# HI-ComputerVision/uni-encoder-code

Measured on AMD Instinct MI355X. Metric: img/s fwd+bwd Swin-L 1024x2048 bs=2 per GPU, higher is better.
Workload: dtype bf16; 1 GPU; BASELINE configs[2]: full OneFormer (Swin-L ws12 backbone + MSDeformAttn pixel decoder + 150-query masked-attention decoder), 1024x2048, fwd+bwd, synthetic loss; global_batch=2, parallelism=dp1, mode=eval() (train_mode reported separately with --full)

## Files before the change

include/uenc.h:

```cpp
#ifndef UENC_H
#define UENC_H
#include <stdint.h>

#ifdef __cplusplus
extern "C" {
#endif

#define UENC_F32 0
#define UENC_BF16 1

#ifndef UENC_STREAM_T
#define UENC_STREAM_T void*
#endif
typedef UENC_STREAM_T uenc_stream_t;

#define UENC_EPI_NONE 0
#define UENC_EPI_GELU 1
#define UENC_EPI_RELU 2
#define UENC_EPI_RESIDUAL 3
#define UENC_EPI_MUL_DGELU 4
#define UENC_EPI_MUL_DRELU 5

int uenc_version(void);
const char* uenc_arch(void);

int uenc_cast_f32_bf16(const float* src, void* dst, long n , uenc_stream_t stream);
int uenc_dropout_bf16(const void* in, void* out, long n, unsigned seed, float p, uenc_stream_t stream);
int uenc_cast_transpose_f32_bf16(const float* src , void* dst , int R, int C, uenc_stream_t stream);

int uenc_cast_multi(const void* table, int n, long total_tiles, uenc_stream_t stream);

int uenc_upsample_bilinear(const float* in, float* out, long NC, int Hi, int Wi, int Ho, int Wo, uenc_stream_t stream);

int uenc_attn_mask(const float* logits, uint8_t* mask, long rows, int Hi, int Wi, int Ho, int Wo, uenc_stream_t stream);

int uenc_add_cast_bf16(const float* a, const float* b, void* out, long n, long period, uenc_stream_t stream);
int uenc_msda_prep_fwd(const float* offaw, long ld, const float* ref, int ref_per_image, const int64_t* shapes, float* loc,
                       float* aw, long rows, int Lq, int M, int L, int P, uenc_stream_t stream);
int uenc_msda_prep_bwd(const float* dloc, const float* daw, const float* aw, const int64_t* shapes, void* doffaw, long ld,
                       long rows, int Lq, int M, int L, int P, uenc_stream_t stream);
int uenc_segment_colsum(const void* x16, long ld, int cols, const int64_t* seg_start, int nseg, long rows_per_image, int images,
                        float* out, uenc_stream_t stream);
// ... 287 lines not shown
```

uni-encoder-code_amd/csrc/fpn_nearest.hip:

```cpp
#include "common.h"

struct NrP {
    const void* a; int a_f32;
    const void* prev; int prev_f32;
    void* out; int out_f32;
    const void* dy; int dy_f32;
    float* dprev;
    int B, H, W, Hs, Ws, C;
};

__device__ __forceinline__ float4 nr_ld4(const void* base, int is_f32, long idx) {
    if (is_f32) return *(const float4*)((const float*)base + idx);
    const bf16x4 v = *(const bf16x4*)((const bf16*)base + idx);
    return make_float4((float)v[0], (float)v[1], (float)v[2], (float)v[3]);
}

__device__ __forceinline__ int nearest_src(int dst, float scale, int n_in) { return min((int)floorf((float)dst * scale), n_in - 1); }

__global__ __launch_bounds__(256) void merge_nearest_fwd_kernel(NrP p) {
    const int cqn = p.C >> 2;
    const long total = (long)p.B * p.H * p.W * cqn;
    const float sy = (float)p.Hs / (float)p.H, sx = (float)p.Ws / (float)p.W;
    for (long t = (long)blockIdx.x * 256 + threadIdx.x; t < total; t += (long)gridDim.x * 256) {
        const int cq = (int)(t % cqn);
// ... 20 lines not shown
    if (i == n_in - 1) hi = n_out - 1;
    lo = lo < 0 ? 0 : lo;
    hi = hi > n_out - 1 ? n_out - 1 : hi;
}

__global__ __launch_bounds__(256) void merge_nearest_bwd_kernel(NrP p) {
    const int cqn = p.C >> 2;
    const long total = (long)p.B * p.Hs * p.Ws * cqn;
    const float sy = (float)p.Hs / (float)p.H, sx = (float)p.Ws / (float)p.W;
    for (long t = (long)blockIdx.x * 256 + threadIdx.x; t < total; t += (long)gridDim.x * 256) {
        const int cq = (int)(t % cqn);
        long r = t / cqn;
        const int j = (int)(r % p.Ws); r /= p.Ws;
        const int i = (int)(r % p.Hs);
        const int b = (int)(r / p.Hs);
        int ylo, yhi, xlo, xhi;
        nearest_range(i, p.Hs, p.H, sy, ylo, yhi);
        nearest_range(j, p.Ws, p.W, sx, xlo, xhi);
        float4 acc = make_float4(0.f, 0.f, 0.f, 0.f);
        for (int oy = ylo; oy <= yhi; ++oy) {
            if (nearest_src(oy, sy, p.Hs) != i) continue;
            for (int ox = xlo; ox <= xhi; ++ox) {
                if (nearest_src(ox, sx, p.Ws) != j) continue;
                const float4 d = nr_ld4(p.dy, p.dy_f32, (((long)b * p.H + oy) * p.W + ox) * p.C + cq * 4);
                acc.x += d.x; acc.y += d.y; acc.z += d.z; acc.w += d.w;
            }
        }
        *(float4*)(p.dprev + t * 4) = acc;
    }
}

static bool nr_dtype(int d) { return d == UENC_F32 || d == UENC_BF16; }

extern "C" int uenc_merge_nearest_tokens_fwd(const void* a, int a_dtype, const void* prev, int prev_dtype, void* out, int out_dtype, int B,
                                             int H, int W, int Hs, int Ws, int C, hipStream_t stream) {
    UENC_CHECK_ARG(a && prev && out && B > 0 && H > 0 && W > 0 && Hs > 0 && Ws > 0 && C > 0 && C % 4 == 0);
    UENC_CHECK_ARG(nr_dtype(a_dtype) && nr_dtype(prev_dtype) && nr_dtype(out_dtype));
    UENC_CHECK_ARG(((uintptr_t)a & (a_dtype == UENC_F32 ? 15 : 7)) == 0 && ((uintptr_t)prev & (prev_dtype == UENC_F32 ? 15 : 7)) == 0 &&
                   ((uintptr_t)out & (out_dtype == UENC_F32 ? 15 : 7)) == 0);
    NrP p{a, a_dtype == UENC_F32, prev, prev_dtype == UENC_F32, out, out_dtype == UENC_F32, nullptr, 0, nullptr, B, H, W, Hs, Ws, C};
    const long total = (long)B * H * W * (C / 4);
    long blocks = (total + 255) / 256;
    if (blocks > 16384) blocks = 16384;
    hipLaunchKernelGGL(merge_nearest_fwd_kernel, dim3((unsigned)blocks), dim3(256), 0, stream, p);
    UENC_LAUNCH_RET();
}

extern "C" int uenc_merge_nearest_tokens_bwd(const void* dy, int dy_dtype, float* dprev, int B, int H, int W, int Hs, int Ws, int C,
                                             hipStream_t stream) {
    UENC_CHECK_ARG(dy && dprev && B > 0 && H > 0 && W > 0 && Hs > 0 && Ws > 0 && C > 0 && C % 4 == 0);
    UENC_CHECK_ARG(nr_dtype(dy_dtype) && ((uintptr_t)dy & (dy_dtype == UENC_F32 ? 15 : 7)) == 0 && ((uintptr_t)dprev & 15) == 0);
    NrP p{nullptr, 0, nullptr, 0, nullptr, 0, dy, dy_dtype == UENC_F32, dprev, B, H, W, Hs, Ws, C};
    const long total = (long)B * Hs * Ws * (C / 4);
    long blocks = (total + 255) / 256;
    if (blocks > 16384) blocks = 16384;
    hipLaunchKernelGGL(merge_nearest_bwd_kernel, dim3((unsigned)blocks), dim3(256), 0, stream, p);
    UENC_LAUNCH_RET();
}
```

uni-encoder-code_amd/csrc/gemm.hip:

```cpp
#include "common.h"
#include "prof.h"

#define BM 128
#define BN 128
#define BK 64
#define GEMM_THREADS 256

enum { EPI_NONE = 0, EPI_GELU = 1, EPI_RELU = 2, EPI_RESIDUAL = 3, EPI_MUL_DGELU = 4, EPI_MUL_DRELU = 5 };

struct GemmNT {
    const void* A; int a_f32; long lda;
    const bf16* W; long ldw;
    void* C; long ldc;
    const float* bias;
    const void* aux; long ldaux;
    bf16* aux_out; long ldaux_out;
    int M, N, K;
    int tiles_m, tiles_n;
    int klen;
    int atomic;
    int persist;
    float alpha;
    const float* sample_scale; float inv_rows;
    long part_stride;
    int splits;
    long bsA, bsW, bsC;
    const float* ln_gamma; const float* ln_beta; float* ln_y32; bf16* ln_y16; float2* ln_stats; float ln_eps;
};

__device__ __forceinline__ float nt_alpha(const GemmNT& p, int m) {
    return p.sample_scale == nullptr ? p.alpha : p.alpha * p.sample_scale[(int)(((float)m + 0.5f) * p.inv_rows)];
}

__device__ __forceinline__ int lds_off(int row, int chunk) { return row * 128 + ((chunk ^ ((row >> 1) & 7)) << 4); }

template <bool F32>
__device__ __forceinline__ u32x4 load_row8(const void* base, long ld, int row, int nrows, int k, int kend, int K) {
    const bool ok = (row < nrows) && (k < kend);
    const int rc = min(row, nrows - 1), kc = min(k, K - 8);
    u32x4 v;
    if (F32) {
        const float* p = (const float*)base + (long)rc * ld + kc;
        const float4 a = *(const float4*)p, b = *(const float4*)(p + 4);
        const bf16x8 r = cvt8(a, b);
        v = *(const u32x4*)&r;
    } else {
        v = *(const u32x4*)((const bf16*)base + (long)rc * ld + kc);
    }
    const u32x4 z = {0u, 0u, 0u, 0u};
    return ok ? v : z;
}

template <int EPI, int OUT_F32>
__global__ __launch_bounds__(GEMM_THREADS) void gemm_nt_kernel(GemmNT p) {
    __shared__ __attribute__((aligned(16))) unsigned char smem[2 * (BM + BN) * BK * 2];
    if (blockIdx.z > 0) {
        p.A = (const char*)p.A + (long)blockIdx.z * p.bsA * (p.a_f32 ? 4 : 2);
        p.W += (long)blockIdx.z * p.bsW;
        p.C = (char*)p.C + (long)blockIdx.z * p.bsC * (OUT_F32 ? 4 : 2);
    }
// ... 621 lines not shown
                bf16x8 sv;
                if (full8) sv = *(const bf16x8*)ap;
                else {
                    const bf16x4 q4 = *(const bf16x4*)ap;
#pragma unroll
                    for (int r = 0; r < 4; ++r) { sv[r] = q4[r]; sv[4 + r] = (bf16)0.f; }
                }
#pragma unroll
                for (int r = 0; r < 8; ++r)
                    v[r] = (EPI == EPI_MUL_DGELU) ? v[r] * dgelu_f((float)sv[r]) : (((float)sv[r] > 0.f) ? v[r] : 0.f);
            }
            if (OUT_F32) {
                float* c = (float*)p.C + (long)m * p.ldc + n;
                if (EPI == EPI_NONE && p.atomic) {
#pragma unroll
                    for (int r = 0; r < 8; ++r)
                        if (r < 4 || full8) atomicAdd(c + r, v[r]);
                } else {
                    *(float4*)c = make_float4(v[0], v[1], v[2], v[3]);
                    if (full8) *(float4*)(c + 4) = make_float4(v[4], v[5], v[6], v[7]);
                }
            } else {
                bf16x8 o;
#pragma unroll
                for (int r = 0; r < 8; ++r) o[r] = (bf16)v[r];
                bf16* c = (bf16*)p.C + (long)m * p.ldc + n;
                if (full8) *(bf16x8*)c = o;
                else { bf16x4 q4; q4[0] = o[0]; q4[1] = o[1]; q4[2] = o[2]; q4[3] = o[3]; *(bf16x4*)c = q4; }
            }
        }
    }
}

template <int EPI, int OUT_F32, int BNT = BN2, bool LN = false>
__global__ __launch_bounds__(T2) void gemm_nt256_kernel(GemmNT p) {
    static_assert(BNT == 256 || BNT == 192, "tile width");
    constexpr int NI = BNT / 64;
    constexpr int NB1 = NI - 2;
    constexpr int BNW = BNT / 4;
    extern __shared__ __attribute__((aligned(16))) unsigned char smem[];
    const int t = threadIdx.x, lane = t & 63, wave = t >> 6;
    const int wm = wave >> 2, wn = wave & 3;
    const int ntiles_all = p.tiles_m * p.tiles_n;
    int pos = blockIdx.x;
    bool prefetched = false;
    const bf16* src[4][2];
    for (;;) {
    const int tile = xcd_remap(pos, ntiles_all);
    const int mt = tile / p.tiles_n, nt = tile - mt * p.tiles_n;
    const int m0 = mt * BM2, n0 = nt * BNT;
    const int pos_next = pos + (int)gridDim.x;
    const bool has_next = p.persist && pos_next < ntiles_all;
    const int kt0 = blockIdx.y * (p.klen / BK);
    const int nkt = min(p.K / BK - kt0, p.klen / BK);
    if (OUT_F32 && p.part_stride > 0) p.C = (float*)p.C + (long)blockIdx.y * p.part_stride;

    f32x4 acc[4][8];
#pragma unroll
    for (int i = 0; i < 4; ++i)
#pragma unroll
        for (int j = 0; j < 8; ++j) acc[i][j] = (f32x4){0.f, 0.f, 0.f, 0.f};

    typedef __attribute__((address_space(3))) void lds_void;
    const int fr = lane & 15, fg = lane >> 4;
    {
        auto set_src = [&](int mm0, int nn0) {
#pragma unroll
            for (int q = 0; q < 2; ++q) {
                const int lr = q * 64 + (t >> 3), slot = t & 7;
                const int chunk = slot ^ ((lr >> 1) & 7);
                const int ra = (lr >> 6) * 128 + (lr & 63), rb = (lr >> 5) * BNW + (lr & 31);
                const int rb1 = NB1 == 2 ? rb + 32 : (lr >> 4) * BNW + 32 + (lr & 15);
                src[0][q] = (const bf16*)p.A + (long)min(mm0 + ra, p.M - 1) * p.lda + chunk * 8 + (long)kt0 * BK;
                src[3][q] = (const bf16*)p.A + (long)min(mm0 + ra + 64, p.M - 1) * p.lda + chunk * 8 + (long)kt0 * BK;
                src[1][q] = p.W + (long)min(nn0 + rb, p.N - 1) * p.ldw + chunk * 8 + (long)kt0 * BK;
                src[2][q] = p.W + (long)min(nn0 + rb1, p.N - 1) * p.ldw + chunk * 8 + (long)kt0 * BK;
            }
        };
        if (!prefetched) set_src(m0, n0);
        const int U = 4 * nkt;
        auto issue = [&](int o, int tile) {
            unsigned char* dst = smem + (tile & 1) * 65536 + (o == 0 ? 0 : o == 1 ? 32768 : o == 2 ? 49152 : 16384) + wave * 1024;
#pragma unroll
            for (int q = 0; q < 2; ++q)
                if (q == 0 || o != 2 || NB1 == 2)
                    __builtin_amdgcn_global_load_lds(src[o][q] + (long)tile * BK, (lds_void*)(dst + q * 8192), 16, 0, 0);
        };
        auto inflight = [&](int first) {
            if (NB1 == 2) return 2 * min(max(U - first, 0), 4);
            int n = 0;
#pragma unroll
            for (int k = 0; k < 4; ++k)
                if (first + k < U) n += (((first + k) & 3) == 2) ? 1 : 2;
            return n;
        };
        auto prologue = [&]() {
            if (BNT == 192) { issue(0, 0); issue(1, 0); issue(3, 0); issue(2, 0); }
            else { issue(0, 0); issue(1, 0); issue(2, 0); issue(3, 0); }
            if (U > 4) { issue(0, 1); issue(1, 1); }
        };
        if (!prefetched) prologue();
        if (BNT == 192) wait_vmcnt_upto8(3 + (U > 4 ? 4 : 0));
        else wait_vmcnt_upto8(inflight(2));
        __builtin_amdgcn_s_barrier();
        if (wm == 1) __builtin_amdgcn_s_barrier();

        const int aoff = lds_off(wm * 64 + fr, fg), boff = lds_off(wn * 32 + fr, fg);
        const int boff1 = NB1 == 2 ? boff : lds_off(wn * 16 + fr, fg);
        if constexpr (BNT == 192) {
        bf16x8 af0[4][2], af1[4][2], b0[2][2], b1[1][2];
        for (int T = 0; T < nkt; ++T) {
            const unsigned char* buf = smem + (T & 1) * 65536;
            const bool n1 = T + 1 < nkt, n2 = T + 2 < nkt;
#pragma unroll
            for (int i = 0; i < 2; ++i)
#pragma unroll
                for (int ks = 0; ks < 2; ++ks) b0[i][ks] = *(const bf16x8*)(buf + 32768 + i * 2048 + (boff ^ (ks << 6)));
            __builtin_amdgcn_sched_barrier(0);
#pragma unroll
// ... 243 lines not shown
    }
    if (!OUT_F32) {
        nt_epilogue_direct<EPI>(p, acc, m0, n0 + wn * 64, fr, fg, true);
        return;
    }
    __syncthreads();
    nt_epilogue_staged<EPI, OUT_F32, T3, 1, 4, LN>(p, acc, smem, m0, n0, 0, wn, t, fr, fg, true);
}

template <int EPI, int OUT_F32, bool LN = false>
static int launch_nt128(GemmNT& p, hipStream_t stream) {
    p.tiles_m = (p.M + BM3 - 1) / BM3; p.tiles_n = (p.N + BN3 - 1) / BN3;
    static bool attr_set = false;
    if (!attr_set) {
        hipError_t e = hipFuncSetAttribute((const void*)gemm_nt128_kernel<EPI, OUT_F32, LN>, hipFuncAttributeMaxDynamicSharedMemorySize, 3 * STAGE3);
        if (e != hipSuccess) return (int)e;
        attr_set = true;
    }
    p.persist = 0;
    hipLaunchKernelGGL((gemm_nt128_kernel<EPI, OUT_F32, LN>), dim3(p.tiles_m * p.tiles_n), dim3(T3), 3 * STAGE3, stream, p);
    return UENC_OK;
}

static int nt_cu_count() {
    static int ncu = 0;
    if (ncu == 0) {
        int dev = 0, v = 0;
        if (hipGetDevice(&dev) == hipSuccess && hipDeviceGetAttribute(&v, hipDeviceAttributeMultiprocessorCount, dev) == hipSuccess && v >= 8) ncu = v / 8 * 8;
        else ncu = 256;
    }
    return ncu;
}

template <int EPI, int OUT_F32, int BNT = BN2, bool LN = false>
static int launch_nt256(GemmNT& p, hipStream_t stream) {
    p.tiles_m = (p.M + BM2 - 1) / BM2; p.tiles_n = (p.N + BNT - 1) / BNT;
    static bool attr_set = false;
    if (!attr_set) {
        hipError_t e = hipFuncSetAttribute((const void*)gemm_nt256_kernel<EPI, OUT_F32, BNT, LN>, hipFuncAttributeMaxDynamicSharedMemorySize, 131072);
        if (e != hipSuccess) return (int)e;
        attr_set = true;
    }
    const int ncu = nt_cu_count();
    const int ntiles = p.tiles_m * p.tiles_n;
    p.persist = (p.splits == 1 && ntiles > ncu) ? 1 : 0;
    hipLaunchKernelGGL((gemm_nt256_kernel<EPI, OUT_F32, BNT, LN>), dim3(p.persist ? ncu : ntiles, p.splits), dim3(T2), 131072, stream, p);
    return UENC_OK;
}

template <int EPI, int OUT_F32>
static int launch_nt_tile128(GemmNT& p, int batch, hipStream_t stream) {
    p.tiles_m = (p.M + BM - 1) / BM; p.tiles_n = (p.N + BN - 1) / BN;
    hipLaunchKernelGGL((gemm_nt_kernel<EPI, OUT_F32>), dim3(p.tiles_m * p.tiles_n, p.splits, batch), dim3(GEMM_THREADS), 0, stream, p);
    return UENC_OK;
}

template <int EPI, int OUT_F32, int A_F32>
static int launch_nt_fewrow_a(GemmNT& p, int nr, hipStream_t stream) {
    const dim3 block(GEMM_THREADS);
    if (nr == 1) {
        p.tiles_m = (p.M + 63) / 64; p.tiles_n = (p.N + 63) / 64;
        hipLaunchKernelGGL((gemm_nt_fewrow_kernel<EPI, OUT_F32, A_F32, 1, 2, 2>), dim3(p.tiles_m * p.tiles_n), block, 0, stream, p);
        return UENC_OK;
    }
    p.tiles_n = (p.N + 31) / 32;
    if ((long)((p.M + 31) / 32) * p.tiles_n * 2 >= nt_cu_count()) {
        p.tiles_m = (p.M + 31) / 32;
        hipLaunchKernelGGL((gemm_nt_fewrow_kernel<EPI, OUT_F32, A_F32, 4, 2, 2>), dim3(p.tiles_m * p.tiles_n), block, 0, stream, p);
    } else {
        p.tiles_m = (p.M + 15) / 16;
        hipLaunchKernelGGL((gemm_nt_fewrow_kernel<EPI, OUT_F32, A_F32, 4, 1, 2>), dim3(p.tiles_m * p.tiles_n), block, 0, stream, p);
    }
    return UENC_OK;
}

template <int EPI, int OUT_F32>
static int launch_nt_fewrow(GemmNT& p, int nr, hipStream_t stream) {
    return p.a_f32 ? launch_nt_fewrow_a<EPI, OUT_F32, 1>(p, nr, stream) : launch_nt_fewrow_a<EPI, OUT_F32, 0>(p, nr, stream);
}
// ... 66 lines not shown
    UENC_CHECK_ARG(a_dtype == UENC_F32 ? (lda % 4 == 0) : (lda % 8 == 0));
    UENC_CHECK_ARG(((uintptr_t)A & 15) == 0 && ((uintptr_t)W & 15) == 0 && ((uintptr_t)C & 15) == 0);
    UENC_CHECK_ARG(epilogue >= EPI_NONE && epilogue <= EPI_MUL_DRELU);
    UENC_CHECK_ARG(tile == 0 || tile == UENC_NT_TILE_256X256 || tile == UENC_NT_TILE_256X192 || tile == UENC_NT_TILE_128X256);
    if (epilogue >= EPI_RESIDUAL) UENC_CHECK_ARG(aux != nullptr && ldaux % 4 == 0);
    if (splitk < 1) splitk = 1;
    if (splitk > 1 || accumulate) UENC_CHECK_ARG(c_dtype == UENC_F32 && epilogue == EPI_NONE);
    GemmNT p;
    p.A = A; p.a_f32 = (a_dtype == UENC_F32); p.lda = lda;
    p.W = (const bf16*)W; p.ldw = ldw;
    p.C = C; p.ldc = ldc; p.bias = bias; p.aux = aux; p.ldaux = ldaux;
    p.aux_out = (bf16*)aux_out; p.ldaux_out = ldaux_out;
    p.M = M; p.N = N; p.K = K;
    p.tiles_m = 0; p.tiles_n = 0; p.persist = 0;
    const int kt = (K + BK - 1) / BK;
    if (splitk > kt) splitk = kt;
    p.klen = ((kt + splitk - 1) / splitk) * BK;
    splitk = (K + p.klen - 1) / p.klen;
    p.atomic = (splitk > 1 || accumulate) ? 1 : 0;
    p.part_stride = 0; p.splits = splitk;
    const bool partials = part_stride > 0;
    if (partials) {
        UENC_CHECK_ARG(c_dtype == UENC_F32 && epilogue == EPI_NONE && !accumulate && bias == nullptr && batch == 1 && part_stride % 4 == 0);
        p.atomic = 0; p.part_stride = part_stride;
    }
    p.alpha = alpha;
    p.sample_scale = nullptr; p.inv_rows = 0.f;
    if (sample_scale != nullptr) {
        UENC_CHECK_ARG(rows_per_sample > 0 && !p.atomic && !partials && batch == 1 && M < (1 << 22));
        p.sample_scale = sample_scale; p.inv_rows = 1.0f / (float)rows_per_sample;
    }
    p.bsA = bsA; p.bsW = bsW; p.bsC = bsC;
    p.ln_gamma = nullptr; p.ln_beta = nullptr; p.ln_y32 = nullptr; p.ln_y16 = nullptr; p.ln_stats = nullptr; p.ln_eps = 0.f;

    const bool summed = p.atomic || partials;
    const NtRoute route = nt_route(M, N, K, batch, a_dtype, lda, c_dtype, epilogue, summed, p.klen, splitk, ln != nullptr, tile);
    if (route == NT_REFUSED) return UENC_EINVAL;
    const bool dma_kernel = route == NT_HALF || route == NT_256 || route == NT_192;
    if (c_dtype == UENC_F32) UENC_CHECK_ARG(epilogue == EPI_NONE || epilogue == EPI_RESIDUAL || epilogue == EPI_RELU);
    else UENC_CHECK_ARG(epilogue != EPI_RESIDUAL || dma_kernel);
    if (ln != nullptr) {
        UENC_CHECK_ARG(epilogue == EPI_RESIDUAL && c_dtype == UENC_F32 && !summed && N <= 256 && N % 8 == 0 && ldc == N &&
                       ln->gamma && ln->beta && (ln->y32 || ln->y16));
        UENC_CHECK_ARG((((uintptr_t)ln->gamma | (uintptr_t)ln->beta | (uintptr_t)ln->y32 | (uintptr_t)ln->y16) & 15) == 0 && ((uintptr_t)ln->stats & 7) == 0);
        p.ln_gamma = ln->gamma; p.ln_beta = ln->beta; p.ln_y32 = ln->y32; p.ln_y16 = (bf16*)ln->y16; p.ln_stats = (float2*)ln->stats; p.ln_eps = ln->eps;
    }

    const bool prof = uenc_prof_on();
    if (prof) {
        const double mn = (double)M * N;
        double bytes = (double)M * K * (a_dtype == UENC_F32 ? 4 : 2) + (double)N * K * 2 + mn * (c_dtype == UENC_F32 ? 4 : 2);
        if (epilogue == EPI_RESIDUAL) bytes += mn * 4;
        if (epilogue == EPI_MUL_DGELU || epilogue == EPI_MUL_DRELU) bytes += mn * 2;
        if (aux_out != nullptr) bytes += mn * 2;
        uenc_prof_begin(route == NT_HALF ? UENC_PROF_GEMM_NT128 : dma_kernel ? UENC_PROF_GEMM_NT256 : UENC_PROF_GEMM_NT, 2.0 * batch * M * (double)N * K, stream,
                        batch * bytes);
    }
    int rc = UENC_EINVAL;
    if (ln != nullptr) {
        rc = route == NT_HALF ? launch_nt128<EPI_RESIDUAL, 1, true>(p, stream)
                              : route == NT_192 ? launch_nt256<EPI_RESIDUAL, 1, 192, true>(p, stream) : launch_nt256<EPI_RESIDUAL, 1, BN2, true>(p, stream);
    } else {
        switch (epilogue * 2 + (c_dtype == UENC_F32 ? 1 : 0)) {
#define NT_CASE(E, F) case (E) * 2 + (F): rc = launch_nt<E, F>(route, p, batch, stream); break
            NT_CASE(EPI_NONE, 1); NT_CASE(EPI_RESIDUAL, 1); NT_CASE(EPI_RELU, 1);
            NT_CASE(EPI_NONE, 0); NT_CASE(EPI_GELU, 0); NT_CASE(EPI_RELU, 0); NT_CASE(EPI_MUL_DGELU, 0); NT_CASE(EPI_MUL_DRELU, 0);
            NT_CASE(EPI_RESIDUAL, 0);
#undef NT_CASE
            default: break;
        }
    }
    if (prof) uenc_prof_end(stream);
    if (rc != UENC_OK) return rc;
    UENC_LAUNCH_RET();
}

extern "C" int uenc_gemm_nt(const void* A, int a_dtype, long lda, const void* W, long ldw, void* C, int c_dtype, long ldc,
                            int M, int N, int K, const float* bias, int epilogue, const void* aux, long ldaux,
                            void* aux_out, long ldaux_out, float alpha, int splitk, int accumulate, hipStream_t stream) {
    return gemm_nt_impl(A, a_dtype, lda, W, ldw, C, c_dtype, ldc, M, N, K, bias, epilogue, aux, ldaux, aux_out, ldaux_out, alpha, splitk,
                        accumulate, 1, 0, 0, 0, stream);
}

extern "C" int uenc_gemm_nt_tile(const void* A, int a_dtype, long lda, const void* W, long ldw, void* C, int c_dtype, long ldc,
                                 int M, int N, int K, const float* bias, int epilogue, const void* aux, long ldaux,
                                 void* aux_out, long ldaux_out, float alpha, int splitk, int accumulate, int tile, hipStream_t stream) {
    return gemm_nt_impl(A, a_dtype, lda, W, ldw, C, c_dtype, ldc, M, N, K, bias, epilogue, aux, ldaux, aux_out, ldaux_out, alpha, splitk,
                        accumulate, 1, 0, 0, 0, stream, 0, nullptr, 0, nullptr, tile);
}

extern "C" int uenc_gemm_nt_scaled(const void* A, int a_dtype, long lda, const void* W, long ldw, void* C, int c_dtype, long ldc,
                                   int M, int N, int K, const float* bias, int epilogue, const void* aux, long ldaux,
                                   void* aux_out, long ldaux_out, float alpha, const float* sample_scale, int rows_per_sample,
                                   hipStream_t stream) {
    UENC_CHECK_ARG(sample_scale != nullptr && rows_per_sample > 0);
    return gemm_nt_impl(A, a_dtype, lda, W, ldw, C, c_dtype, ldc, M, N, K, bias, epilogue, aux, ldaux, aux_out, ldaux_out, alpha, 1,
                        0, 1, 0, 0, 0, stream, 0, sample_scale, rows_per_sample);
}

extern "C" int uenc_gemm_nt_ln(const void* A, int a_dtype, long lda, const void* W, long ldw, void* C, long ldc, int M, int N, int K, const float* bias,
                               const void* residual, long ldres, const float* gamma, const float* beta, float eps, float* y32, void* y16, float* stats,
                               hipStream_t stream) {
    UENC_CHECK_ARG(residual != nullptr);
    NtLn ln = {gamma, beta, y32, y16, stats, eps};
    return gemm_nt_impl(A, a_dtype, lda, W, ldw, C, UENC_F32, ldc, M, N, K, bias, EPI_RESIDUAL, residual, ldres, nullptr, 0, 1.0f, 1, 0, 1, 0, 0, 0, stream, 0,
                        nullptr, 0, &ln);
}

extern "C" int uenc_gemm_nt_splits(int K, int splitk) {
    const int kt = (K + BK - 1) / BK;
    if (splitk < 1) splitk = 1;
    if (splitk > kt) splitk = kt;
    const int klen = (kt + splitk - 1) / splitk;
    return (kt + klen - 1) / klen;
}

extern "C" int uenc_gemm_nt_partials(const void* A, int a_dtype, long lda, const void* W, long ldw, float* P, long ldp, long part_stride,
                                     int M, int N, int K, float alpha, int splitk, hipStream_t stream) {
    UENC_CHECK_ARG(splitk >= 1 && uenc_gemm_nt_splits(K, splitk) == splitk && part_stride >= (long)(M - 1) * ldp + N);
    return gemm_nt_impl(A, a_dtype, lda, W, ldw, P, UENC_F32, ldp, M, N, K, nullptr, EPI_NONE, nullptr, 0, nullptr, 0, alpha, splitk, 0, 1, 0, 0,
                        0, stream, part_stride);
// ... 467 lines not shown
```

uni-encoder-code_amd/uenc/kernels.py:

```python
import collections
import ctypes
import itertools
import operator
import os
from typing import Optional

import numpy as np
import torch

from . import capi
from .capi import BF16, F32, check, dt, lib, ptr, stream_ptr

EPI_NONE, EPI_GELU, EPI_RELU, EPI_RESIDUAL, EPI_MUL_DGELU, EPI_MUL_DRELU = (
    capi.EPI_NONE, capi.EPI_GELU, capi.EPI_RELU, capi.EPI_RESIDUAL, capi.EPI_MUL_DGELU, capi.EPI_MUL_DRELU)
_H = capi.CONSTANTS
NT_TILE_256X256, NT_TILE_256X192, NT_TILE_128X256 = (_H["UENC_NT_TILE_" + t] for t in ("256X256", "256X192", "128X256"))


EXACT = os.environ.get("UENC_EXACT", "0") == "1"


def adt():
    return torch.float32 if EXACT else torch.bfloat16


def _odt(dtype):
    return torch.float32 if (EXACT and dtype == torch.bfloat16) else dtype


def _mat(t: torch.Tensor, name: str):
    if not t.is_cuda:
        raise capi.UencError(f"{name} must live on the GPU")
    if t.dim() != 2 or t.stride(1) != 1:
        raise capi.UencError(f"{name} must be 2-D with unit inner stride, got {tuple(t.shape)} / {t.stride()}")
    return t


CAPTURE_ARENA = None


def upload_table(arr, device, pinned: bool = True) -> torch.Tensor:
    raw = arr.view(np.uint8).reshape(-1)
    if CAPTURE_ARENA is None:
        if not pinned:
            return torch.from_numpy(raw.copy()).to(device)
        return torch.from_numpy(raw).pin_memory().to(device, non_blocking=True)
    host, off = CAPTURE_ARENA[0], CAPTURE_ARENA[1]
    n = int(raw.size)
    end = off + -(-n // 256) * 256
# ... 769 lines not shown
def merge_nearest_tokens_bwd(dy, Hs: int, Ws: int):
    B, H, W, C = dy.shape
    assert dy.is_contiguous()
    out = torch.empty((B, Hs, Ws, C), dtype=torch.float32, device=dy.device)
    check(lib.uenc_merge_nearest_tokens_bwd(dy.data_ptr(), dt(dy), out.data_ptr(), B, H, W, Hs, Ws, C, stream_ptr()),
          "merge_nearest_tokens_bwd")
    return out


def im2col3x3(x16):
    B, H, W, C = x16.shape
    if EXACT and x16.dtype == torch.float32:
        return im2col3x3(x16.contiguous().view(torch.bfloat16)).view(torch.float32)
    assert x16.dtype == torch.bfloat16 and x16.is_contiguous()
    col = torch.empty((B * H * W, 9 * C), dtype=torch.bfloat16, device=x16.device)
    check(lib.uenc_im2col3x3(x16.data_ptr(), col.data_ptr(), B, H, W, C, stream_ptr()), "im2col3x3")
    return col


def col2im3x3(dcol, B: int, H: int, W: int, C: int):
    if EXACT and dcol.dtype == torch.float32:
        d = dcol.view(B, H, W, 9, C)
        dxp = dcol.new_zeros((B, H + 2, W + 2, C))
        for t in range(9):
            ky, kx = divmod(t, 3)
            dxp[:, ky:ky + H, kx:kx + W] += d[:, :, :, t]
        return dxp[:, 1:1 + H, 1:1 + W].contiguous()
    assert dcol.dtype == torch.bfloat16 and dcol.is_contiguous() and dcol.numel() == B * H * W * 9 * C
    dx = torch.empty((B, H, W, C), dtype=torch.bfloat16, device=dcol.device)
    check(lib.uenc_col2im3x3(dcol.data_ptr(), dx.data_ptr(), B, H, W, C, stream_ptr()), "col2im3x3")
    return dx


def add_cast_bf16(a: torch.Tensor, b: torch.Tensor) -> torch.Tensor:
    assert a.dtype == torch.float32 and b.dtype == torch.float32 and a.is_contiguous() and b.is_contiguous()
    if EXACT:
        return (a.view(-1, b.numel()) + b.view(1, -1)).view(a.shape)
    out = torch.empty(a.shape, dtype=torch.bfloat16, device=a.device)
    check(lib.uenc_add_cast_bf16(a.data_ptr(), b.data_ptr(), out.data_ptr(), a.numel(), b.numel(), stream_ptr()), "add_cast_bf16")
    return out


def msda_prep_fwd(offaw: torch.Tensor, ref: torch.Tensor, shapes: torch.Tensor, B: int, Lq: int, M: int, L: int, P: int):
    assert offaw.dtype == torch.float32 and offaw.stride(1) == 1 and ref.dtype == torch.float32 and ref.is_contiguous()
    loc = torch.empty((B, Lq, M, L, P, 2), dtype=torch.float32, device=offaw.device)
    aw = torch.empty((B, Lq, M, L, P), dtype=torch.float32, device=offaw.device)
    check(lib.uenc_msda_prep_fwd(offaw.data_ptr(), offaw.stride(0), ref.data_ptr(), int(ref.shape[0] != 1), shapes.data_ptr(),
                                 loc.data_ptr(), aw.data_ptr(), B * Lq, Lq, M, L, P, stream_ptr()), "msda_prep_fwd")
    return loc, aw


def msda_prep_bwd(dloc, daw, aw, shapes, ncols: int):
    B, Lq, M, L, P, _ = dloc.shape
    assert dloc.is_contiguous() and daw.is_contiguous() and aw.is_contiguous() and ncols == 3 * M * L * P
    if EXACT:
        norm = torch.stack([shapes[:, 1], shapes[:, 0]], -1).to(torch.float32).view(1, 1, 1, L, 1, 2)
        doff = (dloc / norm).reshape(B * Lq, 2 * M * L * P)
        a, g = aw.view(B * Lq, M, L * P), daw.view(B * Lq, M, L * P)
        dlog = (a * (g - (a * g).sum(-1, keepdim=True))).reshape(B * Lq, M * L * P)
        return torch.cat([doff, dlog], 1).contiguous()
    out = torch.empty((B * Lq, ncols), dtype=torch.bfloat16, device=dloc.device)
    check(lib.uenc_msda_prep_bwd(dloc.data_ptr(), daw.data_ptr(), aw.data_ptr(), shapes.data_ptr(), out.data_ptr(), ncols, B * Lq, Lq,
                                 M, L, P, stream_ptr()), "msda_prep_bwd")
    return out


# ... 683 lines not shown
```

uni-encoder-code_amd/uenc/ops.py:

```python
import copy
import dataclasses
import os
import weakref
from typing import List, NamedTuple, Optional, Sequence, Tuple, Union

import numpy as np
import torch
import torch.nn.functional as F

from . import kernels as K
from .capi import check, lib, stream_ptr

BF16, F32 = torch.bfloat16, torch.float32


class CastPiece(NamedTuple):
    owner: int; src_off: int; dst_off: int
    rows: int; cols: int; tr: int


class RelposPlan(NamedTuple):
    ws: int; nH: int


# ... 1290 lines not shown
    @staticmethod
    def backward(ctx, dy):
        x, gamma, beta, stats = ctx.saved_tensors
        G, relu, add_hw, src_shape, dx_dtype = ctx.cfg
        dy = dy if dy.is_contiguous() else dy.contiguous()
        train = gamma.requires_grad
        dx = K.groupnorm_tokens_bwd(dy, x, gamma.detach(), beta.detach(), stats, G, relu=relu,
                                    dgamma=grad_buf(gamma) if train else None, dbeta=grad_buf(beta) if train else None,
                                    dx_dtype=dx_dtype)
        if train:
            _tn_notify(gamma, beta)
        dsrc = None
        if src_shape is not None and ctx.needs_input_grad[6]:
            B, Hs, Ws, C = src_shape
            dsrc = K.upsample_bilinear_tokens_bwd(dy.view(B, add_hw[0], add_hw[1], C), Hs, Ws)
        return dx, None, None, None, None, None, dsrc, None, None, None


def group_norm_tokens(x, gn, *, relu=False, add_src=None, add_hw=None, out_dtype=F32, dx_dtype=BF16):
    assert not (relu and add_src is not None)
    return GroupNormTokensFn.apply(x, gn.weight, gn.bias, gn.num_groups, gn.eps, relu, add_src, add_hw, out_dtype, dx_dtype)


def _conv_wmat(weight, tag, transposed=False, pad8=False):
    def make():
        w = weight.detach().permute(0, 2, 3, 1).reshape(weight.shape[0], -1)
        if pad8:
            w = F.pad(w, (0, -w.shape[1] % 8, 0, -w.shape[0] % 8))
        w = w.contiguous()
        return K.cast_transpose_bf16(w) if transposed else K.cast_bf16(w), None
    return CACHE._get((weight,), tag + "t" if transposed else tag, make)


def _conv_dy(dy, M, Co):
    dy2 = dy.reshape(M, Co)
    dy2 = dy2 if dy2.is_contiguous() else dy2.contiguous()
    return dy2 if dy2.dtype == K.adt() else K.cast_bf16(dy2.float())


def _conv_wgrad(dy2, col, weight, bias, gemm=None):
    Co, C, kh, kw = weight.shape
    dw = torch.zeros((dy2.shape[1], col.shape[1]), dtype=F32, device=dy2.device)
    db = torch.zeros((dy2.shape[1],), dtype=F32, device=dy2.device) if bias is not None else None
    (gemm or K.gemm_tn)(dy2, col, dw, db)
    grad_buf(weight).add_(dw[:Co, :kh * kw * C].view(Co, kh, kw, C).permute(0, 3, 1, 2))
    if bias is not None:
        grad_buf(bias).add_(db[:Co])
    _tn_notify(weight, bias)


class Conv3x3Fn(torch.autograd.Function):

    @staticmethod
    def _wgrad_gemm(dy2, col, dw, db):
        M, Co = dy2.shape
        if M % 64 == 0 and Co % 8 == 0 and not K.EXACT:
            tile = 256 if Co % 256 == 0 else 128
            WgradQueue.launch(tile, [WgradWork.of(dy2, col, dw, None, tile, max(1, M // 16384))], dy2.device)
        else:
            K.gemm_tn(dy2, col, dw, None)

    @staticmethod
    def forward(ctx, x, weight, bias=None):
        B, H, W, C = x.shape
        x16 = x if x.dtype == K.adt() else x.to(K.adt())
        col = K.im2col3x3(x16 if x16.is_contiguous() else x16.contiguous())
        out = K.gemm_nt(col, _conv_wmat(weight, "c3"), bias=None if bias is None else bias.detach(), out_dtype=F32)
        ctx.save_for_backward(col, weight, bias)
        ctx.shape = (B, H, W, C)
        ctx.in_dtype = x.dtype
        ctx.ordered = _ORDERED
        return out.view(B, H * W, weight.shape[0])

    @staticmethod
    def backward(ctx, dy):
        col, weight, bias = ctx.saved_tensors
        B, H, W, C = ctx.shape
        dy2 = _conv_dy(dy, B * H * W, weight.shape[0])
        dx = None
        if ctx.needs_input_grad[0]:
            dcol = K.gemm_nt(dy2, _conv_wmat(weight, "c3", True))
            dx = K.col2im3x3(dcol, B, H, W, C)
            dx = dx if dx.dtype == ctx.in_dtype else dx.to(ctx.in_dtype)
        if weight.requires_grad:
            _conv_wgrad(dy2, col, weight, bias, _tn_ordered if ctx.ordered else (Conv3x3Fn._wgrad_gemm if bias is None else None))
        return dx, None, None


def conv3x3(x_nhwc, weight, bias=None):
    return Conv3x3Fn.apply(x_nhwc, weight, bias)


class _SubCtx:
    saved_tensors = ()

    def __init__(self, needs):
        self.needs_input_grad = tuple(needs)

    def save_for_backward(self, *tensors):
        self.saved_tensors = tensors


def _save_inner(ctx, *subs):
    ctx.save_for_backward(*(t for c in subs for t in c.saved_tensors))
    ctx.counts = tuple(len(c.saved_tensors) for c in subs)
    for c in subs:
        del c.saved_tensors
    ctx.subs = subs


# ... 520 lines not shown
```

Measured before the change: 31.50 img/s.

## Replace im2col 3x3 convolution with implicit GEMM over padded NHWC input

Adds a padded-copy kernel and a CONV variant of the 256-wide NT GEMM that computes per-tap row offsets into a zero-padded NHWC buffer, so forward, dgrad (reversed taps with transposed weights) and wgrad (nine shifted TN GEMMs) no longer materialize a 9x im2col matrix. This removes the im2col/col2im passes and their large memory traffic, and the saved activation for backward becomes the padded input instead of the column matrix. The new entry points reuse existing C APIs through special dtype codes, and the path is restricted to channel counts that are multiples of 64 and to non-exact, non-ordered mode.

Result: no change. 31.18 img/s, median of 2 (-1.0%).

```diff
diff --git a/include/uenc.h b/include/uenc.h
--- a/include/uenc.h
+++ b/include/uenc.h
@@ -8,6 +8,8 @@
 
 #define UENC_F32 0
 #define UENC_BF16 1
+#define UENC_BF16_CONV3X3 2
+#define UENC_BF16_CONV3X3_REV 3
 
 #ifndef UENC_STREAM_T
 #define UENC_STREAM_T void*
diff --git a/uni-encoder-code_amd/csrc/fpn_nearest.hip b/uni-encoder-code_amd/csrc/fpn_nearest.hip
--- a/uni-encoder-code_amd/csrc/fpn_nearest.hip
+++ b/uni-encoder-code_amd/csrc/fpn_nearest.hip
@@ -76,8 +76,57 @@
 
 static bool nr_dtype(int d) { return d == UENC_F32 || d == UENC_BF16; }
 
+template <bool F32>
+__global__ __launch_bounds__(256) void conv3x3_pad_kernel(const void* __restrict__ in, bf16* __restrict__ out, int B, int H, int W, int C,
+                                                          long rows, long Mp) {
+    const int c8n = C >> 3, W2 = W + 2, H2 = H + 2;
+    const long G = W + 3, total = rows * c8n;
+    for (long t = (long)blockIdx.x * 256 + threadIdx.x; t < total; t += (long)gridDim.x * 256) {
+        const int c8 = (int)(t % c8n);
+        const long pr = t / c8n - G;
+        u32x4 v = {0u, 0u, 0u, 0u};
+        if (pr >= 0 && pr < Mp) {
+            const int xx = (int)(pr % W2);
+            const long r = pr / W2;
+            const int yy = (int)(r % H2), b = (int)(r / H2);
+            if (yy >= 1 && yy <= H && xx >= 1 && xx <= W) {
+                const long src = (((long)b * H + yy - 1) * W + xx - 1) * C + c8 * 8;
+                if (F32) {
+                    const float* p = (const float*)in + src;
+                    const bf16x8 q = cvt8(*(const float4*)p, *(const float4*)(p + 4));
+                    v = *(const u32x4*)&q;
+                } else {
+                    v = *(const u32x4*)((const bf16*)in + src);
+                }
+            }
+        }
+        *(u32x4*)(out + t * 8) = v;
+    }
+}
+
+static long conv3x3_pad_rows(int B, int H, int W) {
+    const long Mp = (long)B * (H + 2) * (W + 2);
+    return 2 * ((long)W + 3) + (Mp + 63) / 64 * 64;
+}
+
+static int conv3x3_pad(const void* in, int in_dtype, void* out, int B, int H, int W, int C, hipStream_t stream) {
+    UENC_CHECK_ARG(in && out && B > 0 && H > 0 && W > 0 && C > 0 && C % 8 == 0 && (((uintptr_t)in | (uintptr_t)out) & 15) == 0);
+    UENC_CHECK_ARG(in_dtype == UENC_F32 || in_dtype == UENC_BF16);
+    const long rows = conv3x3_pad_rows(B, H, W), Mp = (long)B * (H + 2) * (W + 2);
+    const long total = rows * (C / 8);
+    long blocks = (total + 255) / 256;
+    if (blocks > 65536) blocks = 65536;
+    if (in_dtype == UENC_F32) hipLaunchKernelGGL(conv3x3_pad_kernel<true>, dim3((unsigned)blocks), dim3(256), 0, stream, in, (bf16*)out, B, H, W, C, rows, Mp);
+    else hipLaunchKernelGGL(conv3x3_pad_kernel<false>, dim3((unsigned)blocks), dim3(256), 0, stream, in, (bf16*)out, B, H, W, C, rows, Mp);
+    UENC_LAUNCH_RET();
+}
+
 extern "C" int uenc_merge_nearest_tokens_fwd(const void* a, int a_dtype, const void* prev, int prev_dtype, void* out, int out_dtype, int B,
                                              int H, int W, int Hs, int Ws, int C, hipStream_t stream) {
+    if (out_dtype == UENC_BF16_CONV3X3) {
+        UENC_CHECK_ARG(prev == nullptr);
+        return conv3x3_pad(a, a_dtype, out, B, H, W, C, stream);
+    }
     UENC_CHECK_ARG(a && prev && out && B > 0 && H > 0 && W > 0 && Hs > 0 && Ws > 0 && C > 0 && C % 4 == 0);
     UENC_CHECK_ARG(nr_dtype(a_dtype) && nr_dtype(prev_dtype) && nr_dtype(out_dtype));
     UENC_CHECK_ARG(((uintptr_t)a & (a_dtype == UENC_F32 ? 15 : 7)) == 0 && ((uintptr_t)prev & (prev_dtype == UENC_F32 ? 15 : 7)) == 0 &&
diff --git a/uni-encoder-code_amd/csrc/gemm.hip b/uni-encoder-code_amd/csrc/gemm.hip
--- a/uni-encoder-code_amd/csrc/gemm.hip
+++ b/uni-encoder-code_amd/csrc/gemm.hip
@@ -26,6 +26,7 @@
     int splits;
     long bsA, bsW, bsC;
     const float* ln_gamma; const float* ln_beta; float* ln_y32; bf16* ln_y16; float2* ln_stats; float ln_eps;
+    int cv_H, cv_W, cv_C, cv_kpt, cv_magic, cv_step;
 };
 
 __device__ __forceinline__ float nt_alpha(const GemmNT& p, int m) {
@@ -713,7 +714,7 @@
     }
 }
 
-template <int EPI, int OUT_F32, int BNT = BN2, bool LN = false>
+template <int EPI, int OUT_F32, int BNT = BN2, bool LN = false, bool CONV = false>
 __global__ __launch_bounds__(T2) void gemm_nt256_kernel(GemmNT p) {
     static_assert(BNT == 256 || BNT == 192, "tile width");
     constexpr int NI = BNT / 64;
@@ -752,8 +753,17 @@
                 const int chunk = slot ^ ((lr >> 1) & 7);
                 const int ra = (lr >> 6) * 128 + (lr & 63), rb = (lr >> 5) * BNW + (lr & 31);
                 const int rb1 = NB1 == 2 ? rb + 32 : (lr >> 4) * BNW + 32 + (lr & 15);
+                if constexpr (CONV) {
+                    auto prow = [&](int m) {
+                        const int hw = p.cv_H * p.cv_W, b = m / hw, rem = m - b * hw, y = rem / p.cv_W, x = rem - y * p.cv_W;
+                        return (long)((b * (p.cv_H + 2) + y + 1) * (p.cv_W + 2) + x + 1) * p.cv_C;
+                    };
+                    src[0][q] = (const bf16*)p.A + prow(min(mm0 + ra, p.M - 1)) + chunk * 8;
+                    src[3][q] = (const bf16*)p.A + prow(min(mm0 + ra + 64, p.M - 1)) + chunk * 8;
+                } else {
                 src[0][q] = (const bf16*)p.A + (long)min(mm0 + ra, p.M - 1) * p.lda + chunk * 8 + (long)kt0 * BK;
                 src[3][q] = (const bf16*)p.A + (long)min(mm0 + ra + 64, p.M - 1) * p.lda + chunk * 8 + (long)kt0 * BK;
+                }
                 src[1][q] = p.W + (long)min(nn0 + rb, p.N - 1) * p.ldw + chunk * 8 + (long)kt0 * BK;
                 src[2][q] = p.W + (long)min(nn0 + rb1, p.N - 1) * p.ldw + chunk * 8 + (long)kt0 * BK;
             }
@@ -762,10 +772,18 @@
         const int U = 4 * nkt;
         auto issue = [&](int o, int tile) {
             unsigned char* dst = smem + (tile & 1) * 65536 + (o == 0 ? 0 : o == 1 ? 32768 : o == 2 ? 49152 : 16384) + wave * 1024;
+            long koff = (long)tile * BK;
+            if constexpr (CONV) {
+                if (o == 0 || o == 3) {
+                    const int tap = (tile * p.cv_magic) >> 16, kc = tile - tap * p.cv_kpt;
+                    const int ky = (tap * 11) >> 5, kx = tap - 3 * ky;
+                    koff = (long)(((ky - 1) * (p.cv_W + 2) + (kx - 1)) * p.cv_step * p.cv_C + kc * BK);
+                }
+            }
 #pragma unroll
             for (int q = 0; q < 2; ++q)
                 if (q == 0 || o != 2 || NB1 == 2)
-                    __builtin_amdgcn_global_load_lds(src[o][q] + (long)tile * BK, (lds_void*)(dst + q * 8192), 16, 0, 0);
+                    __builtin_amdgcn_global_load_lds(src[o][q] + koff, (lds_void*)(dst + q * 8192), 16, 0, 0);
         };
         auto inflight = [&](int first) {
             if (NB1 == 2) return 2 * min(max(U - first, 0), 4);
@@ -1075,19 +1093,19 @@
     return ncu;
 }
 
-template <int EPI, int OUT_F32, int BNT = BN2, bool LN = false>
+template <int EPI, int OUT_F32, int BNT = BN2, bool LN = false, bool CONV = false>
 static int launch_nt256(GemmNT& p, hipStream_t stream) {
     p.tiles_m = (p.M + BM2 - 1) / BM2; p.tiles_n = (p.N + BNT - 1) / BNT;
     static bool attr_set = false;
     if (!attr_set) {
-        hipError_t e = hipFuncSetAttribute((const void*)gemm_nt256_kernel<EPI, OUT_F32, BNT, LN>, hipFuncAttributeMaxDynamicSharedMemorySize, 131072);
+        hipError_t e = hipFuncSetAttribute((const void*)gemm_nt256_kernel<EPI, OUT_F32, BNT, LN, CONV>, hipFuncAttributeMaxDynamicSharedMemorySize, 131072);
         if (e != hipSuccess) return (int)e;
         attr_set = true;
     }
     const int ncu = nt_cu_count();
     const int ntiles = p.tiles_m * p.tiles_n;
     p.persist = (p.splits == 1 && ntiles > ncu) ? 1 : 0;
-    hipLaunchKernelGGL((gemm_nt256_kernel<EPI, OUT_F32, BNT, LN>), dim3(p.persist ? ncu : ntiles, p.splits), dim3(T2), 131072, stream, p);
+    hipLaunchKernelGGL((gemm_nt256_kernel<EPI, OUT_F32, BNT, LN, CONV>), dim3(p.persist ? ncu : ntiles, p.splits), dim3(T2), 131072, stream, p);
     return UENC_OK;
 }
 
@@ -1220,6 +1238,7 @@
     }
     p.bsA = bsA; p.bsW = bsW; p.bsC = bsC;
     p.ln_gamma = nullptr; p.ln_beta = nullptr; p.ln_y32 = nullptr; p.ln_y16 = nullptr; p.ln_stats = nullptr; p.ln_eps = 0.f;
+    p.cv_H = p.cv_W = p.cv_C = p.cv_kpt = p.cv_magic = p.cv_step = 0;
 
     const bool summed = p.atomic || partials;
     const NtRoute route = nt_route(M, N, K, batch, a_dtype, lda, c_dtype, epilogue, summed, p.klen, splitk, ln != nullptr, tile);
@@ -1270,11 +1289,68 @@
                         accumulate, 1, 0, 0, 0, stream);
 }
 
+static int conv3x3_gemm(const void* xp, int B, int H, int W, int C, const void* Wmat, long ldw, void* out, int out_dtype, long ldc,
+                        int N, const float* bias, int reverse, int tile, hipStream_t stream);
+
 extern "C" int uenc_gemm_nt_tile(const void* A, int a_dtype, long lda, const void* W, long ldw, void* C, int c_dtype, long ldc,
                                  int M, int N, int K, const float* bias, int epilogue, const void* aux, long ldaux,
                                  void* aux_out, long ldaux_out, float alpha, int splitk, int accumulate, int tile, hipStream_t stream) {
+    if (a_dtype == UENC_BF16_CONV3X3 || a_dtype == UENC_BF16_CONV3X3_REV) {
+        UENC_CHECK_ARG(M > 0 && N > 0 && K > 0 && K % 9 == 0 && lda > 0 && lda % (K / 9) == 0 && lda / (K / 9) >= 3 && ldaux > 0);
+        UENC_CHECK_ARG(aux == nullptr && aux_out == nullptr && epilogue == EPI_NONE && alpha == 1.0f && splitk <= 1 && accumulate == 0);
+        const long Cch = K / 9, Wd = lda / Cch - 2, H = ldaux;
+        UENC_CHECK_ARG(Wd < (1L << 30) && H < (1L << 30) && (long)M % (H * Wd) == 0);
+        return conv3x3_gemm(A, (int)(M / (H * Wd)), (int)H, (int)Wd, (int)Cch, W, ldw, C, c_dtype, ldc, N, bias, a_dtype == UENC_BF16_CONV3X3_REV, tile, stream);
+    }
     return gemm_nt_impl(A, a_dtype, lda, W, ldw, C, c_dtype, ldc, M, N, K, bias, epilogue, aux, ldaux, aux_out, ldaux_out, alpha, splitk,
                         accumulate, 1, 0, 0, 0, stream, 0, nullptr, 0, nullptr, tile);
+}
+
+static long conv_guard_rows(int W) { return (long)W + 3; }
+
+static NtRoute conv3x3_route(int B, int H, int W, int C, int N, int out_dtype, int tile) {
+    if (B <= 0 || H <= 0 || W <= 0 || C <= 0 || N <= 0 || C % 64 != 0 || N % 8 != 0 || C > 4096) return NT_REFUSED;
+    if (out_dtype != UENC_F32 && out_dtype != UENC_BF16) return NT_REFUSED;
+    if (tile != 0 && tile != UENC_NT_TILE_256X256 && tile != UENC_NT_TILE_256X192) return NT_REFUSED;
+    const long M = (long)B * H * W, Mp = (long)B * (H + 2) * (W + 2);
+    if (M >= (1L << 31) || Mp >= (1L << 31) || conv_guard_rows(W) * C >= (1L << 31)) return NT_REFUSED;
+    const int K = 9 * C;
+    if (tile != 0)
+        return N >= 192 ? (tile == UENC_NT_TILE_256X192 ? NT_192 : NT_256) : NT_REFUSED;
+    const NtRoute r = nt_route((int)M, N, K, 1, UENC_BF16, C, out_dtype, EPI_NONE, false, K, 1, false, 0);
+    return (r == NT_256 || r == NT_192) ? r : NT_REFUSED;
+}
+
+static int conv3x3_gemm(const void* xp, int B, int H, int W, int C, const void* Wmat, long ldw, void* out, int out_dtype, long ldc,
+                        int N, const float* bias, int reverse, int tile, hipStream_t stream) {
+    const NtRoute route = conv3x3_route(B, H, W, C, N, out_dtype, tile);
+    if (route == NT_REFUSED) return UENC_EINVAL;
+    if (out == nullptr) return UENC_OK;
+    UENC_CHECK_ARG(xp && Wmat);
+    UENC_CHECK_ARG(ldw % 8 == 0 && ldw >= 9L * C && ldc % 4 == 0 && ldc >= N);
+    UENC_CHECK_ARG(((uintptr_t)xp & 15) == 0 && ((uintptr_t)Wmat & 15) == 0 && ((uintptr_t)out & 15) == 0);
+    GemmNT p;
+    p.A = (const bf16*)xp + conv_guard_rows(W) * C; p.a_f32 = 0; p.lda = C;
+    p.W = (const bf16*)Wmat; p.ldw = ldw;
+    p.C = out; p.ldc = ldc; p.bias = bias; p.aux = nullptr; p.ldaux = 0; p.aux_out = nullptr; p.ldaux_out = 0;
+    p.M = B * H * W; p.N = N; p.K = 9 * C;
+    p.tiles_m = 0; p.tiles_n = 0; p.persist = 0;
+    p.klen = p.K; p.atomic = 0; p.part_stride = 0; p.splits = 1;
+    p.alpha = 1.0f; p.sample_scale = nullptr; p.inv_rows = 0.f;
+    p.bsA = p.bsW = p.bsC = 0;
+    p.ln_gamma = nullptr; p.ln_beta = nullptr; p.ln_y32 = nullptr; p.ln_y16 = nullptr; p.ln_stats = nullptr; p.ln_eps = 0.f;
+    p.cv_H = H; p.cv_W = W; p.cv_C = C; p.cv_kpt = C / BK; p.cv_magic = (65536 + p.cv_kpt - 1) / p.cv_kpt; p.cv_step = reverse ? -1 : 1;
+    const bool prof = uenc_prof_on();
+    if (prof) {
+        const double M = (double)p.M, Mp = (double)B * (H + 2) * (W + 2);
+        uenc_prof_begin(UENC_PROF_GEMM_NT256, 2.0 * M * N * p.K, stream, Mp * C * 2 + (double)N * p.K * 2 + M * N * (out_dtype == UENC_F32 ? 4 : 2));
+    }
+    int rc;
+    if (out_dtype == UENC_F32) rc = route == NT_192 ? launch_nt256<EPI_NONE, 1, 192, false, true>(p, stream) : launch_nt256<EPI_NONE, 1, BN2, false, true>(p, stream);
+    else rc = route == NT_192 ? launch_nt256<EPI_NONE, 0, 192, false, true>(p, stream) : launch_nt256<EPI_NONE, 0, BN2, false, true>(p, stream);
+    if (prof) uenc_prof_end(stream);
+    if (rc != UENC_OK) return rc;
+    UENC_LAUNCH_RET();
 }
 
 extern "C" int uenc_gemm_nt_scaled(const void* A, int a_dtype, long lda, const void* W, long ldw, void* C, int c_dtype, long ldc,
diff --git a/uni-encoder-code_amd/uenc/kernels.py b/uni-encoder-code_amd/uenc/kernels.py
--- a/uni-encoder-code_amd/uenc/kernels.py
+++ b/uni-encoder-code_amd/uenc/kernels.py
@@ -15,6 +15,7 @@
     capi.EPI_NONE, capi.EPI_GELU, capi.EPI_RELU, capi.EPI_RESIDUAL, capi.EPI_MUL_DGELU, capi.EPI_MUL_DRELU)
 _H = capi.CONSTANTS
 NT_TILE_256X256, NT_TILE_256X192, NT_TILE_128X256 = (_H["UENC_NT_TILE_" + t] for t in ("256X256", "256X192", "128X256"))
+BF16_CONV3X3, BF16_CONV3X3_REV = _H["UENC_BF16_CONV3X3"], _H["UENC_BF16_CONV3X3_REV"]
 
 
 EXACT = os.environ.get("UENC_EXACT", "0") == "1"
@@ -850,6 +851,40 @@
     return dx
 
 
+def conv3x3_pad_geometry(B: int, H: int, W: int):
+    Mp = B * (H + 2) * (W + 2)
+    return W + 3, Mp, -(-Mp // 64) * 64
+
+
+def conv3x3_pad(x):
+    B, H, W, C = x.shape
+    assert x.dtype in (torch.float32, torch.bfloat16) and x.is_contiguous() and x.is_cuda
+    G, _, Mr = conv3x3_pad_geometry(B, H, W)
+    xp = torch.empty((2 * G + Mr, C), dtype=torch.bfloat16, device=x.device)
+    check(lib.uenc_merge_nearest_tokens_fwd(x.data_ptr(), dt(x), 0, BF16, xp.data_ptr(), BF16_CONV3X3, B, H, W, 0, 0, C, stream_ptr()), "conv3x3_pad")
+    return xp
+
+
+def conv3x3_gemm_ok(B: int, H: int, W: int, C: int, N: int, out_dtype=torch.float32, tile: int = 0) -> bool:
+    return not EXACT and lib.uenc_gemm_nt_tile(0, BF16_CONV3X3, (W + 2) * C, 0, 9 * C, 0, F32 if out_dtype == torch.float32 else BF16, N, B * H * W, N, 9 * C,
+                                               0, EPI_NONE, 0, H, 0, 0, 1.0, 1, 0, int(tile), 0) == 0
+
+
+def conv3x3_gemm(xp, B: int, H: int, W: int, wmat, *, bias=None, out_dtype=torch.float32, reverse: bool = False, tile: int = 0):
+    G, _, Mr = conv3x3_pad_geometry(B, H, W)
+    C = xp.shape[1]
+    N = wmat.shape[0]
+    assert xp.dtype == torch.bfloat16 and xp.is_contiguous() and xp.shape[0] == 2 * G + Mr
+    assert wmat.dtype == torch.bfloat16 and wmat.shape[1] == 9 * C and wmat.stride(1) == 1
+    if bias is not None:
+        assert bias.dtype == torch.float32 and bias.numel() == N and bias.is_contiguous()
+    out = torch.empty((B * H * W, N), dtype=out_dtype, device=xp.device)
+    check(lib.uenc_gemm_nt_tile(xp.data_ptr(), BF16_CONV3X3_REV if reverse else BF16_CONV3X3, (W + 2) * C, wmat.data_ptr(), wmat.stride(0),
+                                out.data_ptr(), dt(out), N, B * H * W, N, 9 * C, ptr(bias), EPI_NONE, 0, H, 0, 0, 1.0, 1, 0, int(tile), stream_ptr()),
+          "conv3x3_gemm")
+    return out
+
+
 def add_cast_bf16(a: torch.Tensor, b: torch.Tensor) -> torch.Tensor:
     assert a.dtype == torch.float32 and b.dtype == torch.float32 and a.is_contiguous() and b.is_contiguous()
     if EXACT:
diff --git a/uni-encoder-code_amd/uenc/ops.py b/uni-encoder-code_amd/uenc/ops.py
--- a/uni-encoder-code_amd/uenc/ops.py
+++ b/uni-encoder-code_amd/uenc/ops.py
@@ -1346,6 +1346,12 @@
     return CACHE._get((weight,), tag + "t" if transposed else tag, make)
 
 
+def _conv_wmat_dgrad(weight, tag):
+    def make():
+        return K.cast_bf16(weight.detach().permute(1, 2, 3, 0).reshape(weight.shape[1], -1).contiguous()), None
+    return CACHE._get((weight,), tag + "d", make)
+
+
 def _conv_dy(dy, M, Co):
     dy2 = dy.reshape(M, Co)
     dy2 = dy2 if dy2.is_contiguous() else dy2.contiguous()
@@ -1374,22 +1380,65 @@
         else:
             K.gemm_tn(dy2, col, dw, None)
 
+    IMPLICIT = True
+    implicit_calls = 0
+
+    @staticmethod
+    def _implicit_ok(x, weight, bias) -> bool:
+        B, H, W, C = x.shape
+        Co = weight.shape[0]
+        return (Conv3x3Fn.IMPLICIT and not K.EXACT and not _ORDERED and x.is_cuda and x.dtype in (F32, BF16) and C % 64 == 0 and Co % 64 == 0
+                and (bias is None or not weight.requires_grad)
+                and K.conv3x3_gemm_ok(B, H, W, C, Co, F32) and K.conv3x3_gemm_ok(B, H, W, Co, C, x.dtype))
+
+    @staticmethod
+    def _wgrad_implicit(dyp, xp, weight, B, H, W):
+        Co, C = weight.shape[0], weight.shape[1]
+        G, _, Mr = K.conv3x3_pad_geometry(B, H, W)
+        dw = torch.zeros((Co, 9 * C), dtype=F32, device=dyp.device)
+        pad = lambda t: (-(-Co // t) * t) * (-(-C // t) * t)
+        tile = 256 if pad(256) <= 1.3 * pad(128) else 128
+        works = []
+        for tap in range(9):
+            off = (tap // 3 - 1) * (W + 2) + (tap % 3 - 1)
+            works.append(WgradWork.of(dyp[G:G + Mr], xp[G + off:G + off + Mr], dw[:, tap * C:(tap + 1) * C], None, tile, max(1, Mr // 16384)))
+        WgradQueue.launch(tile, works, dyp.device)
+        grad_buf(weight).add_(dw.view(Co, 3, 3, C).permute(0, 3, 1, 2))
+        _tn_notify(weight, None)
+
     @staticmethod
     def forward(ctx, x, weight, bias=None):
         B, H, W, C = x.shape
+        ctx.shape = (B, H, W, C)
+        ctx.in_dtype = x.dtype
+        ctx.ordered = _ORDERED
+        ctx.implicit = Conv3x3Fn._implicit_ok(x, weight, bias)
+        if ctx.implicit:
+            xp = K.conv3x3_pad(x if x.is_contiguous() else x.contiguous())
+            out = K.conv3x3_gemm(xp, B, H, W, _conv_wmat(weight, "c3"), bias=None if bias is None else bias.detach(), out_dtype=F32)
+            ctx.save_for_backward(xp, weight, bias)
+            Conv3x3Fn.implicit_calls += 1
+            return out.view(B, H * W, weight.shape[0])
         x16 = x if x.dtype == K.adt() else x.to(K.adt())
         col = K.im2col3x3(x16 if x16.is_contiguous() else x16.contiguous())
         out = K.gemm_nt(col, _conv_wmat(weight, "c3"), bias=None if bias is None else bias.detach(), out_dtype=F32)
         ctx.save_for_backward(col, weight, bias)
-        ctx.shape = (B, H, W, C)
-        ctx.in_dtype = x.dtype
-        ctx.ordered = _ORDERED
         return out.view(B, H * W, weight.shape[0])
 
     @staticmethod
     def backward(ctx, dy):
         col, weight, bias = ctx.saved_tensors
         B, H, W, C = ctx.shape
+        if ctx.implicit:
+            Co = weight.shape[0]
+            dy4 = dy.reshape(B, H, W, Co)
+            dyp = K.conv3x3_pad(dy4 if dy4.is_contiguous() else dy4.contiguous())
+            dx = None
+            if ctx.needs_input_grad[0]:
+                dx = K.conv3x3_gemm(dyp, B, H, W, _conv_wmat_dgrad(weight, "c3"), out_dtype=ctx.in_dtype, reverse=True).view(B, H, W, C)
+            if weight.requires_grad:
+                Conv3x3Fn._wgrad_implicit(dyp, col, weight, B, H, W)
+            return dx, None, None
         dy2 = _conv_dy(dy, B * H * W, weight.shape[0])
         dx = None
         if ctx.needs_input_grad[0]:
```
